# liuzuxin/FSRL

Hardware: AMD Instinct MI355X
Metric: policy-updates/sec (PPO-Lagrangian update(), SafetyCarCircle-v0 shape, 256x256 MLP, 20k-step buffer) (higher is better)
Workload: dtype f32; 1 GPU; configs[1] PPO-Lag update: repeat 4, clip 0.5, KL stop off, batch 256, N=20000 (20x1000), obs 8/act 2, 256x256; seeds_per_gpu=1, parallelism=independent agents x1

## Files before the change

fsrl_amd/_lib.py:

```python
import ctypes as C
import os

_HERE = os.path.dirname(os.path.abspath(__file__))
LIB_PATH = os.environ.get("FSRL_HIP_LIB") or os.path.join(_HERE, "libfsrl_hip.so")

FSRL_OK, FSRL_EINVAL, FSRL_ENOMEM, FSRL_EHIP, FSRL_ESTATE = 0, -22, -12, -5, -1
PPO_NSTATS = 11
ALGO_PPO_LAG, ALGO_TRPO_LAG, ALGO_CPO, ALGO_SAC_LAG, ALGO_FOCOPS = 0, 1, 2, 3, 4


class Config(C.Structure):
    _fields_ = [("algo", C.c_int32), ("obs_dim", C.c_int32), ("act_dim", C.c_int32),
                ("hidden", C.c_int32), ("n_critics", C.c_int32), ("env_num", C.c_int32),
                ("buffer_size", C.c_int64), ("max_action", C.c_float), ("gamma", C.c_double),
                ("gae_lambda", C.c_double), ("eps_clip", C.c_float), ("dual_clip", C.c_float),
                ("vf_coef", C.c_float), ("max_grad_norm", C.c_float), ("target_kl", C.c_float),
                ("norm_adv", C.c_int32), ("use_lagrangian", C.c_int32), ("lr", C.c_float),
                ("beta1", C.c_float), ("beta2", C.c_float), ("adam_eps", C.c_float), ("recompute_adv", C.c_int32),
                ("unbounded", C.c_int32), ("rew_norm", C.c_int32), ("value_clip", C.c_int32),
                ("hidden1", C.c_int32), ("hidden2", C.c_int32),
                ("n_hidden", C.c_int32), ("hidden_sizes", C.c_int32 * 8), ("force_layered", C.c_int32)]


class ShmEnv(C.Structure):
# ... 72 lines not shown
    "fsrl_store_push": (C.c_int, [_ctx, _i32, C.c_int32, _f, _f, _d, _d, _u8, _u8, _f, _i64, _d, _i32, _i64]),
    "fsrl_store_reset": (C.c_int, [_ctx, C.c_int]),
    "fsrl_store_len": (C.c_int64, [_ctx]),
    "fsrl_store_read": (C.c_int, [_ctx, _i64, C.c_int64, _f, _f, _d, _d, _u8, _u8, _f]),
    "fsrl_store_configure": (C.c_int, [_ctx, C.c_int64, C.c_int32]),
    "fsrl_store_geometry": (C.c_int, [_ctx, _i64, _i32]),
    "fsrl_store_sample0": (C.c_int, [_ctx, _i64, C.c_int64, _i64]),
    "fsrl_actor_forward": (C.c_int, [_ctx, _f, C.c_int32, _f, _f]),
    "fsrl_ppo_begin": (C.c_int, [_ctx, _d, C.c_double, C.c_int32, _i64]),
    "fsrl_ppo_pass": (C.c_int, [_ctx, _i64, C.c_uint64, _i32]),
    "fsrl_ppo_pass_result": (C.c_int, [_ctx, _i32]),
    "fsrl_ppo_end": (C.c_int, [_ctx, _f, C.c_int64, _i64]),
    "fsrl_ppo_update": (C.c_int, [_ctx, _d, C.c_double, C.c_int32, C.c_int32, _i64, C.c_uint64, _f,
                                  C.c_int64, _i64, _i32]),
    "fsrl_ppo_set_plan": (C.c_int, [_ctx, C.c_int32]),
    "fsrl_batch_get": (C.c_int, [_ctx, C.c_char_p, _f, C.c_int64]),
    "fsrl_group_create": (C.c_int, [_P(_ctx), C.c_int32, _P(_ctx)]),
    "fsrl_group_destroy": (C.c_int, [_ctx]),
    "fsrl_group_set_plan": (C.c_int, [_ctx, C.c_int32]),
    "fsrl_group_ppo_update": (C.c_int, [_ctx, _d, _d, C.c_int32, C.c_int32, _P(_i64), C.c_uint64, _P(_f), C.c_int64, _i64,
                                        _i32]),
    "fsrl_group_ppo_update_each": (C.c_int, [_ctx, _d, _d, _i32, _i32, _P(_i64), C.c_uint64, _P(_f), _i64, _i64, _i32]),
    "fsrl_group_collect_step": (C.c_int, [_ctx, _i32, _i32, _f, _f, _d, _d, _u8, _u8, _f, _i64, _d, _i32, _i64, _i32, _f, C.c_int32,
                                          C.c_int32, _f, _f, _f, _f]),
    "fsrl_group_actor_set_resident": (C.c_int, [_ctx, C.c_int32, C.c_double]),
    "fsrl_group_actor_resident_stats": (C.c_int, [_ctx, _i64]),
    "fsrl_group_actor_release": (C.c_int, [_ctx]),
    "fsrl_sac_group_create": (C.c_int, [_P(_ctx), C.c_int32, _P(_ctx)]),
    "fsrl_sac_group_destroy": (C.c_int, [_ctx]),
    "fsrl_sac_group_update": (C.c_int, [_ctx, C.c_int32, _i32, _d, _d]),
# ... 126 lines not shown
```

fsrl_amd/csrc/common.hpp:

```cpp
#pragma once
#include <hip/hip_runtime.h>
#include <stdint.h>

#include "../../include/fsrl_hip.h"

#define FSRL_MAX_NETS (1 + FSRL_MAX_CRITICS)
#define FSRL_TILE_M 16
#define FSRL_DOW 32
#define FSRL_MAX_OBS 128
#define FSRL_MAX_ACT 16
#define FSRL_W1_LDS 16
#define FSRL_RD 64
#define FSRL_RD_LOGP 16
#define FSRL_RD_ADV 17
#define FSRL_RD_RET 21
#define FSRL_RD_VOLD 25
#define FSRL_RD_MEAN 32
#define FSRL_RD_STD 48

typedef float f32x4 __attribute__((ext_vector_type(4)));
typedef float f32x2 __attribute__((ext_vector_type(2)));

struct NetOff {
    int sigma;
// ... 51 lines not shown
#define FSRL_PROBE(sa, n) false
#define FSRL_TS(buf, k) do { } while (0)
#endif

__device__ __forceinline__ void ppo_adam_math(const float g, float& m, float& v, float& p, const PpoStepArgs& sa) {
#pragma clang fp contract(off)
    m = fmaf(sa.one_minus_b1, g - m, m);
    v = v * sa.beta2;
    v = fmaf(sa.one_minus_b2 * g, g, v);
    const float denom = sqrtf(v) / sa.bc2_sqrt + sa.adam_eps;
    p = p + (-sa.step_size * m) / denom;
}

struct CtrlBlock {
    int stopped_after;
    int pad;
    double kl_sum;
    float last_grad_norm;
    float pad2;
};

__device__ __forceinline__ f32x4 mfma_16x16x4(float a, float b, f32x4 c) {
    return __builtin_amdgcn_mfma_f32_16x16x4f32(a, b, c, 0, 0, 0);
}

__device__ __forceinline__ f32x4 mfma_4x4x1(float a, float b, f32x4 c) {
    return __builtin_amdgcn_mfma_f32_4x4x1f32(a, b, c, 0, 0, 0);
}

__device__ __forceinline__ void store4_next(float* p, const f32x4 v) {
    asm volatile("global_store_dwordx4 %0, %1, off sc1\n\ts_nop 1" ::"v"(p), "v"(v) : "memory");
// ... 55 lines not shown
```

fsrl_amd/csrc/fsrl_hip.hip:

```cpp
#include <hip/hip_runtime.h>

#include <climits>
#include <cstddef>
#include <cmath>
#include <cstdarg>
#include <cstdio>
#include <cstdlib>
#include <cstring>
#include <algorithm>
#include <functional>
#include <string>
#include <vector>

#include "kernels_misc.hpp"
#include "kernels_mlp.hpp"
#include "kernels_fb.hpp"
#include "kernels_fbco.hpp"
#include "kernels_wgrad2.hpp"
#include "kernels_wgrad3.hpp"
#include "kernels_layered.hpp"
#include "kernels_focops_group.hpp"
#include "resident_ring.hpp"
#include "host_decisions.hpp"

// ... 74 lines not shown
    double* ret64 = nullptr; int64_t ret64_cap = 0;
    int64_t alloc_rows = 0;
    int active_envs = 0;
    std::vector<EnvBook> env;
    std::vector<uint8_t> h_flags;
    StorePtrs st{};
    static constexpr int STAGE_CAP = 4096;
    Staging stage[2];
    int cur_stage = 0;
    hipEvent_t store_ready = nullptr;

    BatchPtrs b{};
    int* d_indices = nullptr; uint8_t* d_end = nullptr; int* d_seg = nullptr;
    int* h_indices = nullptr; uint8_t* h_end = nullptr; int* h_seg = nullptr;
    float *values = nullptr, *vnext = nullptr, *advs = nullptr, *rets = nullptr, *logp_old = nullptr;
    int64_t N = 0;
    int n_seg = 0;
    bool batch_ready = false;

    int batch_size = 0, mbp_max = 0, n_tiles_max = 0;
    float *A1 = nullptr, *A2 = nullptr, *D1 = nullptr, *D2 = nullptr, *DO = nullptr;
    float *obs_p = nullptr, *rd_p = nullptr;
    float *statp = nullptr, *gsq_part = nullptr;
    int *d_perm = nullptr, *h_perm = nullptr;
    int *d_mbstart = nullptr, *d_mbsize = nullptr, *h_mbplan = nullptr;
    size_t mb_cap = 0;
    std::vector<int> mb_start, mb_size;
    float* d_stats = nullptr; int64_t stats_cap = 0;
    int64_t n_steps = 0;
    int pass_index = 0;
// ... 317 lines not shown
    lay_free(c);
    if (c->h_actor) (void)hipHostFree(c->h_actor);
    if (c->h_done) (void)hipHostFree(c->h_done);
    if (c->h_pa) (void)hipHostFree(c->h_pa);
    if (c->mbstat) (void)hipFree(c->mbstat);
    if (c->d_rms) (void)hipFree(c->d_rms);
    if (c->ret64) (void)hipFree(c->ret64);
    if (c->mu_old) (void)hipFree(c->mu_old);
    if (c->sigma_old) (void)hipFree(c->sigma_old);
    if (c->snap) (void)hipFree(c->snap);
    void* dptrs[] = {c->P, c->M, c->V, c->G, c->ctrl, c->st.obs, c->st.obs_next, c->st.act, c->st.rew,
                     c->st.cost, c->st.flags, c->b.obs, c->b.obs_next, c->b.act, c->b.rew, c->b.cost,
                     c->b.flags, c->d_indices, c->d_end, c->d_seg, c->values, c->vnext, c->advs,
                     c->rets, c->logp_old, c->A1, c->A2, c->D1, c->D2, c->DO, c->obs_p, c->rd_p, c->statp,
                     c->gsq_part, c->d_perm, c->d_mbstart, c->d_mbsize, c->d_stats,
                     c->scratch};
    for (void* p : dptrs) if (p) (void)hipFree(p);
    for (auto& pp : c->parts) if (pp.p) (void)hipFree(pp.p);
    void* hptrs[] = {c->h_ctrl, c->h_indices, c->h_end, c->h_seg, c->h_perm, c->h_mbplan};
    for (void* p : hptrs) if (p) (void)hipHostFree(p);
    for (auto& s : c->stage) {
        if (s.h) (void)hipHostFree(s.h);
        if (s.d) (void)hipFree(s.d);
        if (s.done) (void)hipEventDestroy(s.done);
    }
    for (hipEvent_t e : {c->store_ready, c->ev_a, c->ev_b, c->ev_c, c->perm_copied}) if (e) (void)hipEventDestroy(e);
    for (hipEvent_t e : c->k_ev) (void)hipEventDestroy(e);
    if (c->compute) (void)hipStreamDestroy(c->compute);
    if (c->side) (void)hipStreamDestroy(c->side);
    delete c;
    return 0;
}

extern "C" int fsrl_ctx_create(int device_id, const fsrl_config* cfg, fsrl_ctx** out) {
// ... 43 lines not shown
    CHECK_ARG(!cfg->rew_norm || cfg->algo != FSRL_ALGO_SAC_LAG, "reward_normalization acts on GAE returns: on-policy contexts only");
    int ndev = 0;
    HIPCHK(hipGetDeviceCount(&ndev));
    CHECK_ARG(device_id >= 0 && device_id < ndev, "device %d not present (%d devices)", device_id, ndev);
    HIPCHK(hipSetDevice(device_id));
    int n_cus_probe = 256;
    (void)hipDeviceGetAttribute(&n_cus_probe, hipDeviceAttributeMultiprocessorCount, device_id);
    fsrl_ctx* c = new fsrl_ctx();
    c->cfg = *cfg;
    c->cfg.hidden = Hpad_;
    c->h1 = h1_; c->h2 = h2_;
    c->device = device_id;
    c->n_cus = n_cus_probe > 0 ? n_cus_probe : 256;
    c->probe_tile16 = getenv("FSRL_TILE16") != nullptr;
    c->no_w2b_early = getenv("FSRL_NO_W2B_EARLY") != nullptr;
#ifdef FSRL_PROBES
    { const char* e = getenv("FSRL_DBG_PHASE"); c->probe_phase = e ? atoi(e) : 0; }
    { const char* e = getenv("FSRL_WGRAD_SKIP"); c->probe_wgrad_skip = e ? atoi(e) : 0; }
    c->no_spin = getenv("FSRL_NO_SPIN") != nullptr;
    c->no_xcd_pair = getenv("FSRL_NO_XCD_PAIR") != nullptr;
    c->no_fuse_adam = getenv("FSRL_NO_FUSE_ADAM") != nullptr;
    if (getenv("FSRL_TSTAMP")) {
        (void)hipMalloc(&c->probe_ts, 1024 * 16 * sizeof(unsigned long long));
        (void)hipMemset(c->probe_ts, 0, 1024 * 16 * sizeof(unsigned long long));
    }
#endif
    if (layered) lay_build_layout(c, cfg->hidden_sizes, cfg->n_hidden);
    else build_layout(c);
#define TRY(expr) do { hipError_t _e = (expr); if (_e != hipSuccess) { fail(FSRL_EHIP, "%s failed: %s", #expr, hipGetErrorString(_e)); fsrl_ctx_destroy(c); return FSRL_EHIP; } } while (0)
    TRY(hipStreamCreateWithFlags(&c->compute, hipStreamNonBlocking));
// ... 17 lines not shown
    c->h_flags.assign((size_t)c->alloc_rows, 0);
    const size_t ms = (size_t)c->alloc_rows;
    const int Do = cfg->obs_dim, Da = cfg->act_dim;
    TRY(hipMalloc(&c->st.obs, ms * Do * 4)); TRY(hipMalloc(&c->st.obs_next, ms * Do * 4));
    TRY(hipMalloc(&c->st.act, ms * Da * 4)); TRY(hipMalloc(&c->st.rew, ms * 8));
    TRY(hipMalloc(&c->st.cost, ms * 8)); TRY(hipMalloc(&c->st.flags, ms));
    TRY(hipMalloc(&c->b.obs, ms * Do * 4)); TRY(hipMalloc(&c->b.obs_next, ms * Do * 4));
    TRY(hipMalloc(&c->b.act, ms * Da * 4)); TRY(hipMalloc(&c->b.rew, ms * 8));
    TRY(hipMalloc(&c->b.cost, ms * 8)); TRY(hipMalloc(&c->b.flags, ms));
    TRY(hipMalloc(&c->d_indices, ms * 4)); TRY(hipMalloc(&c->d_end, ms)); TRY(hipMalloc(&c->d_seg, (ms + 2) * 4));
    TRY(hipHostMalloc(&c->h_indices, ms * 4)); TRY(hipHostMalloc(&c->h_end, ms)); TRY(hipHostMalloc(&c->h_seg, (ms + 2) * 4));
    const int C = cfg->n_critics;
    TRY(hipMalloc(&c->values, ms * C * 4)); TRY(hipMalloc(&c->vnext, ms * C * 4));
    TRY(hipMalloc(&c->advs, ms * C * 4)); TRY(hipMalloc(&c->rets, ms * C * 4));
    TRY(hipMalloc(&c->logp_old, ms * 4));
    TRY(hipMalloc(&c->d_perm, ms * 4)); TRY(hipHostMalloc(&c->h_perm, ms * 4));
    TRY(hipMalloc(&c->obs_p, (ms + 32) * Do * 4)); TRY(hipMemsetAsync(c->obs_p, 0, (ms + 32) * Do * 4, c->compute));
    TRY(hipMalloc(&c->rd_p, (ms + 32) * FSRL_RD * 4)); TRY(hipMemsetAsync(c->rd_p, 0, (ms + 32) * FSRL_RD * 4, c->compute));
    TRY(hipStreamSynchronize(c->compute));
    for (auto& s : c->stage) {
        const size_t k = fsrl_ctx::STAGE_CAP;
        TRY(hipHostMalloc(&s.h, k * stage_rec_bytes(Do, Da)));
        TRY(hipMalloc(&s.d, k * stage_rec_bytes(Do, Da)));
        TRY(hipEventCreateWithFlags(&s.done, hipEventDisableTiming));
    }
    TRY(hipEventCreateWithFlags(&c->store_ready, hipEventDisableTiming));
    TRY(hipEventCreate(&c->ev_a)); TRY(hipEventCreate(&c->ev_b)); TRY(hipEventCreate(&c->ev_c));
    TRY(hipEventCreateWithFlags(&c->perm_copied, hipEventDisableTiming));
    CtrlBlock init{INT_MAX, 0, 0.0, 0.0f, 0.0f};
    TRY(hipMemcpy(c->ctrl, &init, sizeof(init), hipMemcpyHostToDevice));
// ... 267 lines not shown
    rc = ensure_scratch(c, total);
    if (rc) return rc;
    std::vector<int> idx(N);
    for (size_t i = 0; i < N; ++i) {
        CHECK_ARG(indices[i] >= 0 && indices[i] < c->maxsize, "index %lld out of range", (long long)indices[i]);
        idx[i] = (int)indices[i];
    }
    char* base = (char*)c->scratch;
    hipStream_t s = c->compute;
    HIPCHK(hipMemcpyAsync(base + o_idx, idx.data(), N * 4, hipMemcpyHostToDevice, s));
    HIPCHK(hipMemsetAsync(base + o_end, 0, N, s));
    BatchPtrs b{(float*)(base + o_obs), (float*)(base + o_nxt), (float*)(base + o_act), (double*)(base + o_rew),
                (double*)(base + o_cost), (uint8_t*)(base + o_fl)};
    const size_t work = N * (2 * Do + Da + 1);
    hipLaunchKernelGGL(batch_gather_kernel, dim3((int)std::min<size_t>(2048, (work + 255) / 256)), dim3(256), 0, s, c->st, b,
                       (const int*)(base + o_idx), (const uint8_t*)(base + o_end), (int)n, (int)Do, (int)Da);
    HIPCHK(hipGetLastError());
    std::vector<uint8_t> fl(N);
    if (obs_out) HIPCHK(hipMemcpyAsync(obs_out, b.obs, N * Do * 4, hipMemcpyDeviceToHost, s));
    if (obs_next_out) HIPCHK(hipMemcpyAsync(obs_next_out, b.obs_next, N * Do * 4, hipMemcpyDeviceToHost, s));
    if (act_out) HIPCHK(hipMemcpyAsync(act_out, b.act, N * Da * 4, hipMemcpyDeviceToHost, s));
    if (rew_out) HIPCHK(hipMemcpyAsync(rew_out, b.rew, N * 8, hipMemcpyDeviceToHost, s));
    if (cost_out) HIPCHK(hipMemcpyAsync(cost_out, b.cost, N * 8, hipMemcpyDeviceToHost, s));
    HIPCHK(hipMemcpyAsync(fl.data(), b.flags, N, hipMemcpyDeviceToHost, s));
    HIPCHK(hipStreamSynchronize(s));
    for (size_t i = 0; i < N; ++i) {
        if (terminated_out) terminated_out[i] = fl[i] & 1;
        if (truncated_out) truncated_out[i] = (fl[i] >> 1) & 1;
    }
    return 0;
}
// ... 7 lines not shown
    }
    return fail(FSRL_EINVAL, "unsupported hidden width %d", H);
}

static int launch_infer(fsrl_ctx* c, const InferArgs& ia, int jobs_y, hipStream_t s) {
    const int tiles = (ia.N + 15) / 16;
    if (tiles == 0) return 0;
    if (c->lay) return lay_infer(c, ia, jobs_y, s);
    return dispatch_H(c->cfg.hidden, [&](auto hc) {
        constexpr int H = decltype(hc)::value;
        const int gx = std::min(tiles, std::max(1, c->n_cus / jobs_y));
        hipLaunchKernelGGL(mlp_infer_kernel<H>, dim3(gx, jobs_y), dim3(4 * H), 0, s, c->P, c->md, ia);
        HIPCHK(hipGetLastError());
        return 0;
    });
}

struct SacState;
static bool ctx_is_replay(const fsrl_ctx* c) { return c->cfg.algo == FSRL_ALGO_SAC_LAG; }
static int sac_actor_launch(fsrl_ctx* c, const float* h_obs, float* h_raw, int k);
static void sac_actor_finish(fsrl_ctx* c, const float* h_raw, int k, float* mu_out, float* sigma_out);
static int sac_raw_cols(const fsrl_ctx* c);
static bool sac_squashes(fsrl_ctx* c);
static bool sac_actor_resident_args(fsrl_ctx* c, const float** P, const ModelDesc** md);

struct PaLayout { unsigned long long* bell; unsigned* done; unsigned* state; float* obs; float* mu; float* sp; };
static PaLayout pa_layout(const fsrl_ctx* c) {
    char* b = (char*)c->h_pa;
    PaLayout l;
    l.bell = (unsigned long long*)b; l.done = (unsigned*)(b + 16); l.state = (unsigned*)(b + 32);
// ... 511 lines not shown
```

fsrl_amd/csrc/host_ppo.inc:

```
static int launch_gae(fsrl_ctx* c);
static int perm_upload(fsrl_ctx* c, int n, const int64_t* perm, uint64_t seed) {
    c->perm_tmp.resize((size_t)n);
    const PermFill pf = perm_fill(c->perm_tmp.data(), n, perm, c->shuffle_rng, seed);
    CHECK_ARG(pf.code != PERM_RANGE, "perm[%d]=%lld out of range", pf.index, pf.value);
    CHECK_ARG(pf.code != PERM_TWICE, "perm is not a permutation: %lld appears twice", pf.value);
    if (c->perm_in_flight) { HIPCHK(hipEventSynchronize(c->perm_copied)); c->perm_in_flight = false; }
    memcpy(c->h_perm, c->perm_tmp.data(), (size_t)n * 4);
    HIPCHK(hipMemcpyAsync(c->d_perm, c->h_perm, (size_t)n * 4, hipMemcpyHostToDevice, c->compute));
    HIPCHK(hipEventRecord(c->perm_copied, c->compute));
    c->perm_in_flight = true;
    return 0;
}

static int ensure_ppo_buffers(fsrl_ctx* c, int B) {
    const int mbp = round_up(2 * B, 32);
    if (mbp <= c->mbp_max) return 0;
    HIPCHK(hipStreamSynchronize(c->compute));
    for (float** p : {&c->A1, &c->A2, &c->D1, &c->D2, &c->DO, &c->statp, &c->gsq_part})
        if (*p) { HIPCHK(hipFree(*p)); *p = nullptr; }
    const int H = c->cfg.hidden, nn = c->md.n_nets;
    const size_t act = (size_t)nn * mbp * H * 4;
    HIPCHK(hipMalloc(&c->A1, act)); HIPCHK(hipMalloc(&c->A2, act));
    HIPCHK(hipMalloc(&c->D1, act)); HIPCHK(hipMalloc(&c->D2, act));
    HIPCHK(hipMalloc(&c->DO, (size_t)nn * mbp * FSRL_DOW * 4));
// ... 25 lines not shown
    for (int i = 0; i < FSRL_MAX_CRITICS; ++i) c->lagr[i] = 0.0;
    if (c->cfg.use_lagrangian && C > 1) {
        CHECK_ARG(lagrangians, "lags and values length must be equal");
        for (int i = 0; i < C - 1; ++i) c->lagr[i] = lagrangians[i];
    }
    c->rescaling = rescaling;
    c->batch_size = batch_size;
    const int64_t n = sample0(c, c->h_indices, c->h_end);
    c->N = n;
    if (n_out) *n_out = n;
    c->n_steps = 0;
    c->pass_index = 0;
    c->in_update = true;
    c->verdict_pending = false;
    c->t_fwdbwd_ms = 0; c->n_fwdbwd = 0; c->k_ev_used = 0;
    CtrlBlock init{INT_MAX, 0, 0.0, 0.0f, 0.0f};
    *c->h_ctrl = init;
    hipStream_t s = c->compute;
    HIPCHK(hipMemcpyAsync(c->ctrl, c->h_ctrl, sizeof(CtrlBlock), hipMemcpyHostToDevice, s));
    if (n == 0) { c->batch_ready = true; return 0; }
    int nseg = 0;
    c->h_seg[nseg++] = 0;
    for (int64_t i = 0; i + 1 < n; ++i) if (c->h_end[i]) c->h_seg[nseg++] = (int)i + 1;
    c->h_seg[nseg] = (int)n;
    HIPCHK(hipEventRecord(c->ev_a, s));
    HIPCHK(hipMemcpyAsync(c->d_indices, c->h_indices, (size_t)n * 4, hipMemcpyHostToDevice, s));
    HIPCHK(hipMemcpyAsync(c->d_end, c->h_end, (size_t)n, hipMemcpyHostToDevice, s));
    HIPCHK(hipMemcpyAsync(c->d_seg, c->h_seg, (size_t)(nseg + 1) * 4, hipMemcpyHostToDevice, s));
    const int Do = c->cfg.obs_dim, Da = c->cfg.act_dim;
    {
        const size_t work = (size_t)n * (2 * Do + Da + 1);
        const int blocks = (int)std::min<size_t>(2048, (work + 255) / 256);
        hipLaunchKernelGGL(batch_gather_kernel, dim3(blocks), dim3(256), 0, s, c->st, c->b, c->d_indices,
                           c->d_end, (int)n, Do, Da);
        HIPCHK(hipGetLastError());
    }
    InferArgs ia{};
    ia.obs = c->b.obs; ia.obs_next = c->b.obs_next; ia.act = c->b.act; ia.flags = c->b.flags;
    ia.values = c->values; ia.vnext = c->vnext; ia.logp_old = c->logp_old; ia.mu_out = nullptr;
    if (c->cfg.algo == FSRL_ALGO_FOCOPS) {
        if (!c->mu_old) {
            HIPCHK(hipMalloc(&c->mu_old, (size_t)c->alloc_rows * Da * 4));
            HIPCHK(hipMalloc(&c->sigma_old, FSRL_MAX_ACT * 4));
        }
        ia.mu_out = c->mu_old;
        HIPCHK(hipMemcpyAsync(c->sigma_old, c->P + c->md.net[0].sigma, (size_t)Da * 4, hipMemcpyDeviceToDevice, s));
    }
    ia.N = (int)n; ia.C = C; ia.max_action = c->cfg.max_action;
    rc = launch_infer(c, ia, 2 * C + 1, s);
    if (rc) return rc;
    c->n_seg = nseg;
    rc = launch_gae(c);
    if (rc) return rc;
    HIPCHK(hipEventRecord(c->ev_b, s));
    split_plan((int)n, batch_size, c->mb_start, c->mb_size);
    const int bs_rows = (int)std::min<int64_t>(batch_size, std::max<int64_t>(n, 1));
    rc = c->lay ? lay_ensure_mb(c, bs_rows) : ensure_ppo_buffers(c, bs_rows);
    if (rc) return rc;
    const size_t nmb = c->mb_start.size();
    if (nmb > c->mb_cap) {
        HIPCHK(hipStreamSynchronize(s));
        if (c->d_mbstart) HIPCHK(hipFree(c->d_mbstart));
        if (c->d_mbsize) HIPCHK(hipFree(c->d_mbsize));
        if (c->h_mbplan) HIPCHK(hipHostFree(c->h_mbplan));
// ... 31 lines not shown
    HIPCHK(hipGetLastError());
    if (c->cfg.rew_norm) {
        hipLaunchKernelGGL(ret_rms_update_kernel, dim3(c->cfg.n_critics), dim3(1024), 0, c->compute, c->ret64, c->d_rms,
                           (int)c->N);
        HIPCHK(hipGetLastError());
    }
    return 0;
}

static int ppo_recompute_advantages(fsrl_ctx* c) {
    const int C = c->cfg.n_critics;
    InferArgs ia{};
    ia.obs = c->b.obs; ia.obs_next = c->b.obs_next; ia.act = nullptr; ia.flags = c->b.flags;
    ia.values = c->values; ia.vnext = c->vnext; ia.logp_old = nullptr; ia.mu_out = nullptr;
    ia.N = (int)c->N; ia.C = C; ia.max_action = c->cfg.max_action;
    int rc = launch_infer(c, ia, 2 * C, c->compute);
    if (rc) return rc;
    return launch_gae(c);
}

static int ensure_stats(fsrl_ctx* c, int64_t steps) {
    if (steps <= c->stats_cap) return 0;
    int64_t cap = std::max<int64_t>(steps, c->stats_cap * 2);
    cap = std::max<int64_t>(cap, 1024);
    float* nw = nullptr;
    HIPCHK(hipMalloc(&nw, (size_t)cap * FSRL_PPO_NSTATS * 4));
    if (c->d_stats) {
        HIPCHK(hipStreamSynchronize(c->compute));
        HIPCHK(hipMemcpy(nw, c->d_stats, (size_t)c->stats_cap * FSRL_PPO_NSTATS * 4, hipMemcpyDeviceToDevice));
        HIPCHK(hipFree(c->d_stats));
    }
// ... 265 lines not shown
    CHECK_ARG(c, "null ctx");
    CHECK_ARG(repeat >= 0, "repeat must be >= 0");
    int64_t n = 0;
    int rc = fsrl_ppo_begin(c, lagrangians, rescaling, batch_size, &n);
    if (rc) return rc;
    if (stopped_pass_out) *stopped_pass_out = -1;
    for (int k = 0; k < repeat; ++k) {
        int32_t stopped = 0;
        rc = fsrl_ppo_pass(c, perms ? perms + (size_t)k * n : nullptr, seed ? seed + k : 0, &stopped);
        if (rc) { c->in_update = false; return rc; }
        if (stopped) { if (stopped_pass_out) *stopped_pass_out = k; break; }
    }
    return fsrl_ppo_end(c, stats_out, cap_steps, n_steps_out);
}

extern "C" int fsrl_batch_get(fsrl_ctx* c, const char* which, float* out, int64_t cap) {
    CHECK_ARG(c && which && out, "null argument");
    if (!c->batch_ready) return fail(FSRL_ESTATE, "no batch: call fsrl_ppo_begin first");
    ENTER_DEV(c);
    const int64_t n = c->N;
    const int C = c->cfg.n_critics;
    const float* src = nullptr;
    int cols = C;
    if (!strcmp(which, "values")) src = c->values;
    else if (!strcmp(which, "rets")) src = c->rets;
    else if (!strcmp(which, "advs")) src = c->advs;
    else if (!strcmp(which, "vnext")) src = c->vnext;
    else if (!strcmp(which, "logp_old")) { src = c->logp_old; cols = 1; }
    else return fail(FSRL_EINVAL, "unknown batch field '%s'", which);
    CHECK_ARG(cap >= n * cols, "out too small");
// ... 8 lines not shown
```

fsrl_amd/csrc/kernels_misc.hpp:

```cpp
#pragma once
#include "common.hpp"

struct StorePtrs {
    float* obs;
    float* obs_next;
    float* act;
    double* rew;
    double* cost;
    uint8_t* flags;
};

__global__ void store_scatter_kernel(StorePtrs st, const uint8_t* __restrict__ recs, const int rec, int k, int Do, int Da) {
    const int per = 2 * Do + Da + 1;
    for (int e = blockIdx.x * blockDim.x + threadIdx.x; e < k * per; e += gridDim.x * blockDim.x) {
        const int row = e / per, f = e - row * per;
        const uint8_t* r = recs + (size_t)row * rec;
        const size_t dst = (size_t)*reinterpret_cast<const int*>(r + 16);
        const float* x = reinterpret_cast<const float*>(r + 24);
        if (f < Do) st.obs[dst * Do + f] = x[f];
        else if (f < 2 * Do) st.obs_next[dst * Do + (f - Do)] = x[f];
        else if (f < 2 * Do + Da) st.act[dst * Da + (f - 2 * Do)] = x[f];
        else {
            st.rew[dst] = *reinterpret_cast<const double*>(r);
            st.cost[dst] = *reinterpret_cast<const double*>(r + 8);
            st.flags[dst] = (uint8_t)*reinterpret_cast<const uint32_t*>(r + 20);
        }
    }
}

struct BatchPtrs {
    float* obs; float* obs_next; float* act; double* rew; double* cost; uint8_t* flags;
};

__global__ void batch_gather_kernel(StorePtrs st, BatchPtrs b, const int* __restrict__ indices,
                                    const uint8_t* __restrict__ end_flag, int n, int Do, int Da) {
    const int per = 2 * Do + Da + 1;
    for (size_t e = (size_t)blockIdx.x * blockDim.x + threadIdx.x; e < (size_t)n * per;
         e += (size_t)gridDim.x * blockDim.x) {
        const int row = (int)(e / per), f = (int)(e - (size_t)row * per);
        const size_t src = (size_t)indices[row];
        if (f < Do) b.obs[(size_t)row * Do + f] = st.obs[src * Do + f];
        else if (f < 2 * Do) b.obs_next[(size_t)row * Do + (f - Do)] = st.obs_next[src * Do + (f - Do)];
        else if (f < 2 * Do + Da) b.act[(size_t)row * Da + (f - 2 * Do)] = st.act[src * Da + (f - 2 * Do)];
        else {
            b.rew[row] = st.rew[src];
            b.cost[row] = st.cost[src];
            b.flags[row] = (uint8_t)((st.flags[src] & 3) | (end_flag[row] ? 4 : 0));
        }
    }
}

struct GaeArgs {
    const float* values;
    const float* vnext;
    const double* rew;
    const double* cost;
    const uint8_t* flags;
    const int* seg_start;
    float* advs;
    float* rets;
    double* adv64;
    int N;
    double gamma, gl;
    const double* rms;
// ... 284 lines not shown
```

fsrl_amd/csrc/kernels_mlp.hpp:

```cpp
#pragma once
#include <type_traits>
#include "common.hpp"

__host__ __device__ constexpr int tile_rows(int R) { return R > 16 ? R : 16; }

template <int H, int ROWS = 16>
struct TileSmem {
    static constexpr int LD = H + 4;
    static constexpr int XK = (ROWS > 16) ? 64 : FSRL_MAX_OBS;
    float xT[XK * ROWS];
    float h1[ROWS * LD];
    float h2[ROWS * LD];
    float d2[ROWS * LD];
    float out[ROWS * FSRL_MAX_ACT];
    float dout[ROWS * FSRL_DOW];
    float rd[ROWS * FSRL_RD];
    float st[ROWS * 4];
    float w3[FSRL_MAX_ACT * H];
    float b1[H], b2[H], b3[FSRL_MAX_ACT], sig[FSRL_MAX_ACT];
    float w1[H * FSRL_W1_LDS];
};

template <int H>
struct TileGeom {
// ... 401 lines not shown
        __syncthreads();
#pragma unroll
        for (int u = 0; u < NX; ++u) {
            const int e = tid + u * NT;
            if (e < 16 * Do) { const int i = div_by_magic((unsigned)e, magic), k = e - i * Do; sm.xT[k * 16 + i] = xn[u]; }
        }
        tile = ntile; row0 = nrow0; n_valid = nn_valid;
    }
    if (a.done) {
        if (tid < min(NT, max(256, (16 * a.raw_cols + 63) & ~63))) __atomic_thread_fence(__ATOMIC_RELEASE);
        __syncthreads();
        if (tid == 0) __hip_atomic_store(a.done + blockIdx.x, a.seq, __ATOMIC_RELAXED, __HIP_MEMORY_SCOPE_SYSTEM);
    }
}

#define PACTOR_BLOCKS 4
struct PActorArgs {
    const float* obs;
    float* mu_out;
    float* sigma_param_out;
    const unsigned long long* bell;
    unsigned* done;
    unsigned* state;
    unsigned gen, last_seq;
    unsigned long long timeout_ticks;
    float max_action;
    int raw_cols;
};
#define PACTOR_EXIT 0xFFFFFFFFu

// ... 988 lines not shown
```

fsrl_amd/engine.py:

```python
import ctypes as C
from dataclasses import dataclass
from typing import Optional, Sequence

import numpy as np

from . import _lib

_f32p, _f64p = C.POINTER(C.c_float), C.POINTER(C.c_double)
_u8p, _i32p, _i64p = C.POINTER(C.c_uint8), C.POINTER(C.c_int32), C.POINTER(C.c_int64)


def _ptr(a, t):
    return a.ctypes.data_as(t) if a is not None else None


@dataclass
class EngineConfig:
    obs_dim: int = 8
    act_dim: int = 2
    hidden: int = 128
    hidden_sizes: Optional[Sequence[int]] = None
    force_layered: bool = False
    n_critics: int = 2
    env_num: int = 20
# ... 341 lines not shown
        return bool(stopped.value)

    def ppo_end(self):
        n = C.c_int64()
        _lib.check(self.lib.fsrl_ppo_end(self._ctx, None, 0, C.byref(n)))
        return n.value

    def ppo_end_stats(self, max_steps: int):
        n = C.c_int64()
        out = np.empty((max(max_steps, 1), _lib.PPO_NSTATS), np.float32)
        _lib.check(self.lib.fsrl_ppo_end(self._ctx, _ptr(out, _f32p), out.shape[0], C.byref(n)))
        return out[:n.value]

    def ppo_set_plan(self, tall_tiles: int = -1):
        _lib.check(self.lib.fsrl_ppo_set_plan(self._ctx, int(tall_tiles)))

    def ppo_update(self, lagrangians, rescaling, batch_size, repeat, perms=None, seed=0):
        n = self.ppo_begin(lagrangians, rescaling, batch_size)
        stopped_pass = -1
        steps_per_pass = max(1, -(-n // max(batch_size, 1)))
        try:
            for k in range(repeat):
                if self.ppo_pass(None if perms is None else perms[k], seed + k if seed else 0):
                    stopped_pass = k
                    break
            stats = self.ppo_end_stats(steps_per_pass * max(repeat, 1))
        except BaseException:
            self.ppo_abort()
            raise
        return stats, stopped_pass
# ... 593 lines not shown
```

include/fsrl_hip.h:

```cpp
#ifndef FSRL_HIP_H
#define FSRL_HIP_H

#include <stdint.h>

#ifdef __cplusplus
extern "C" {
#endif

#define FSRL_OK 0
#define FSRL_EINVAL (-22)
#define FSRL_ENOMEM (-12)
#define FSRL_EHIP (-5)
#define FSRL_ESTATE (-1)

#define FSRL_ALGO_PPO_LAG 0
#define FSRL_ALGO_TRPO_LAG 1
#define FSRL_ALGO_CPO 2
#define FSRL_ALGO_SAC_LAG 3
#define FSRL_ALGO_FOCOPS 4

#define FSRL_MAX_CRITICS 4
#define FSRL_MAX_HIDDEN 8
#define FSRL_MAX_WIDTH 4096
#define FSRL_PPO_NSTATS 11
// ... 110 lines not shown
int fsrl_actor_release(fsrl_ctx* ctx);

int fsrl_store_sizes(const fsrl_ctx* ctx, int64_t* sizes_out, int32_t n);

int fsrl_ppo_begin(fsrl_ctx* ctx, const double* lagrangians, double rescaling,
                   int32_t batch_size, int64_t* n_out);
int fsrl_ppo_pass(fsrl_ctx* ctx, const int64_t* perm, uint64_t seed, int32_t* stopped_out);
int fsrl_ppo_pass_result(fsrl_ctx* ctx, int32_t* stopped_out);
int fsrl_ppo_end(fsrl_ctx* ctx, float* stats_out, int64_t cap_steps, int64_t* n_steps_out);
int fsrl_ppo_abort(fsrl_ctx* ctx);
int fsrl_ppo_update(fsrl_ctx* ctx, const double* lagrangians, double rescaling,
                    int32_t batch_size, int32_t repeat, const int64_t* perms, uint64_t seed,
                    float* stats_out, int64_t cap_steps, int64_t* n_steps_out,
                    int32_t* stopped_pass_out);

int fsrl_ppo_set_plan(fsrl_ctx* ctx, int32_t tall_tiles);

typedef struct fsrl_group fsrl_group;
int fsrl_group_create(fsrl_ctx** ctxs, int32_t k, fsrl_group** out);
int fsrl_group_destroy(fsrl_group* group);
int fsrl_group_set_plan(fsrl_group* group, int32_t tall_tiles);
int fsrl_group_ppo_update(fsrl_group* group, const double* lagrangians, const double* rescaling, int32_t batch_size,
                          int32_t repeat, const int64_t* const* perms, uint64_t seed, float* const* stats_out,
                          int64_t cap_steps, int64_t* n_steps_out, int32_t* stopped_pass_out);
int fsrl_group_ppo_update_each(fsrl_group* group, const double* lagrangians, const double* rescaling, const int32_t* batch_sizes,
                               const int32_t* repeats, const int64_t* const* perms, uint64_t seed, float* const* stats_out,
                               const int64_t* cap_steps, int64_t* n_steps_out, int32_t* stopped_pass_out);
int fsrl_group_collect_step(fsrl_group* group, const int32_t* k, const int32_t* env_ids, const float* obs, const float* act,
                            const double* rew, const double* cost, const uint8_t* terminated, const uint8_t* truncated,
                            const float* obs_next, int64_t* ptr_out, double* ep_rew_out, int32_t* ep_len_out,
// ... 186 lines not shown
```

Before: 130.9 updates/s.

## Reuse next-row critic values for V(s') instead of a second dense critic pass

During PPO batch preparation, the gather kernel now checks, bitwise, whether each row's obs_next equals the next row's obs. Rows where they match (not episode end, not last) take vnext straight from values[i+1] in a small fill kernel. Only the mismatched rows are listed and sent through a sparse critic forward, which cuts the dense inference jobs from 2C+1 to C+1. In exchange, the gather kernel gains ballots, atomics and a stamp array, and an extra kernel launch is added. It also assumes that a forward pass on equal inputs gives bitwise-equal outputs.

```diff
diff --git a/fsrl_amd/_lib.py b/fsrl_amd/_lib.py
--- a/fsrl_amd/_lib.py
+++ b/fsrl_amd/_lib.py
@@ -110,6 +110,7 @@
     "fsrl_ppo_update": (C.c_int, [_ctx, _d, C.c_double, C.c_int32, C.c_int32, _i64, C.c_uint64, _f,
                                   C.c_int64, _i64, _i32]),
     "fsrl_ppo_set_plan": (C.c_int, [_ctx, C.c_int32]),
+    "fsrl_ppo_vnext_uncovered": (C.c_int, [_ctx, _i64]),
     "fsrl_batch_get": (C.c_int, [_ctx, C.c_char_p, _f, C.c_int64]),
     "fsrl_group_create": (C.c_int, [_P(_ctx), C.c_int32, _P(_ctx)]),
     "fsrl_group_destroy": (C.c_int, [_ctx]),
diff --git a/fsrl_amd/csrc/common.hpp b/fsrl_amd/csrc/common.hpp
--- a/fsrl_amd/csrc/common.hpp
+++ b/fsrl_amd/csrc/common.hpp
@@ -89,7 +89,7 @@
 
 struct CtrlBlock {
     int stopped_after;
-    int pad;
+    int vnext_unc;
     double kl_sum;
     float last_grad_norm;
     float pad2;
diff --git a/fsrl_amd/csrc/fsrl_hip.hip b/fsrl_amd/csrc/fsrl_hip.hip
--- a/fsrl_amd/csrc/fsrl_hip.hip
+++ b/fsrl_amd/csrc/fsrl_hip.hip
@@ -112,6 +112,9 @@
     int* d_indices = nullptr; uint8_t* d_end = nullptr; int* d_seg = nullptr;
     int* h_indices = nullptr; uint8_t* h_end = nullptr; int* h_seg = nullptr;
     float *values = nullptr, *vnext = nullptr, *advs = nullptr, *rets = nullptr, *logp_old = nullptr;
+    unsigned* vn_stamp = nullptr; int* vn_list = nullptr; unsigned vn_epoch = 0; int* h_vn_count = nullptr;
+    bool vn_reuse = false;
+    bool no_vnext_reuse = false;
     int64_t N = 0;
     int n_seg = 0;
     bool batch_ready = false;
@@ -459,10 +462,10 @@
                      c->b.flags, c->d_indices, c->d_end, c->d_seg, c->values, c->vnext, c->advs,
                      c->rets, c->logp_old, c->A1, c->A2, c->D1, c->D2, c->DO, c->obs_p, c->rd_p, c->statp,
                      c->gsq_part, c->d_perm, c->d_mbstart, c->d_mbsize, c->d_stats,
-                     c->scratch};
+                     c->scratch, c->vn_stamp, c->vn_list};
     for (void* p : dptrs) if (p) (void)hipFree(p);
     for (auto& pp : c->parts) if (pp.p) (void)hipFree(pp.p);
-    void* hptrs[] = {c->h_ctrl, c->h_indices, c->h_end, c->h_seg, c->h_perm, c->h_mbplan};
+    void* hptrs[] = {c->h_ctrl, c->h_indices, c->h_end, c->h_seg, c->h_perm, c->h_mbplan, c->h_vn_count};
     for (void* p : hptrs) if (p) (void)hipHostFree(p);
     for (auto& s : c->stage) {
         if (s.h) (void)hipHostFree(s.h);
@@ -536,6 +539,7 @@
     c->n_cus = n_cus_probe > 0 ? n_cus_probe : 256;
     c->probe_tile16 = getenv("FSRL_TILE16") != nullptr;
     c->no_w2b_early = getenv("FSRL_NO_W2B_EARLY") != nullptr;
+    c->no_vnext_reuse = getenv("FSRL_NO_VNEXT_REUSE") != nullptr;
 #ifdef FSRL_PROBES
     { const char* e = getenv("FSRL_DBG_PHASE"); c->probe_phase = e ? atoi(e) : 0; }
     { const char* e = getenv("FSRL_WGRAD_SKIP"); c->probe_wgrad_skip = e ? atoi(e) : 0; }
@@ -583,6 +587,8 @@
     TRY(hipMalloc(&c->values, ms * C * 4)); TRY(hipMalloc(&c->vnext, ms * C * 4));
     TRY(hipMalloc(&c->advs, ms * C * 4)); TRY(hipMalloc(&c->rets, ms * C * 4));
     TRY(hipMalloc(&c->logp_old, ms * 4));
+    TRY(hipMalloc(&c->vn_stamp, ms * 4)); TRY(hipMemsetAsync(c->vn_stamp, 0, ms * 4, c->compute)); TRY(hipMalloc(&c->vn_list, ms * 4));
+    TRY(hipHostMalloc(&c->h_vn_count, sizeof(int))); *c->h_vn_count = -1;
     TRY(hipMalloc(&c->d_perm, ms * 4)); TRY(hipHostMalloc(&c->h_perm, ms * 4));
     TRY(hipMalloc(&c->obs_p, (ms + 32) * Do * 4)); TRY(hipMemsetAsync(c->obs_p, 0, (ms + 32) * Do * 4, c->compute));
     TRY(hipMalloc(&c->rd_p, (ms + 32) * FSRL_RD * 4)); TRY(hipMemsetAsync(c->rd_p, 0, (ms + 32) * FSRL_RD * 4, c->compute));
@@ -880,7 +886,7 @@
                 (double*)(base + o_cost), (uint8_t*)(base + o_fl)};
     const size_t work = N * (2 * Do + Da + 1);
     hipLaunchKernelGGL(batch_gather_kernel, dim3((int)std::min<size_t>(2048, (work + 255) / 256)), dim3(256), 0, s, c->st, b,
-                       (const int*)(base + o_idx), (const uint8_t*)(base + o_end), (int)n, (int)Do, (int)Da);
+                       (const int*)(base + o_idx), (const uint8_t*)(base + o_end), (int)n, (int)Do, (int)Da, VnextCover{});
     HIPCHK(hipGetLastError());
     std::vector<uint8_t> fl(N);
     if (obs_out) HIPCHK(hipMemcpyAsync(obs_out, b.obs, N * Do * 4, hipMemcpyDeviceToHost, s));
@@ -918,6 +924,26 @@
         HIPCHK(hipGetLastError());
         return 0;
     });
+}
+
+static int launch_infer_reuse(fsrl_ctx* c, const InferArgs& ia, int n_dense, hipStream_t s) {
+    const int tiles = (ia.N + 15) / 16;
+    if (tiles == 0) return 0;
+    const VnextCover vc{c->vn_stamp, c->vn_list, &c->ctrl->vnext_unc, c->vn_epoch};
+    int rc = dispatch_H(c->cfg.hidden, [&](auto hc) {
+        constexpr int H = decltype(hc)::value;
+        const int64_t want = (int64_t)tiles * n_dense;
+        const int G = (int)std::max<int64_t>(n_dense, std::min<int64_t>(c->n_cus, want));
+        hipLaunchKernelGGL(ppo_infer_kernel<H>, dim3(G), dim3(4 * H), 0, s, c->P, c->md, ia, n_dense, vc.list, vc.count);
+        HIPCHK(hipGetLastError());
+        return 0;
+    });
+    if (rc) return rc;
+    const int work = ia.N * ia.C;
+    hipLaunchKernelGGL(vnext_fill_kernel, dim3((work + 255) / 256), dim3(256), 0, s, vc, ia.values, ia.vnext, ia.flags, ia.N, ia.C,
+                       c->h_vn_count);
+    HIPCHK(hipGetLastError());
+    return 0;
 }
 
 struct SacState;
diff --git a/fsrl_amd/csrc/host_ppo.inc b/fsrl_amd/csrc/host_ppo.inc
--- a/fsrl_amd/csrc/host_ppo.inc
+++ b/fsrl_amd/csrc/host_ppo.inc
@@ -63,6 +63,8 @@
     c->in_update = true;
     c->verdict_pending = false;
     c->t_fwdbwd_ms = 0; c->n_fwdbwd = 0; c->k_ev_used = 0;
+    c->vn_reuse = !c->lay && !c->group && !c->no_vnext_reuse;
+    *c->h_vn_count = (c->vn_reuse && n == 0) ? 0 : -1;
     CtrlBlock init{INT_MAX, 0, 0.0, 0.0f, 0.0f};
     *c->h_ctrl = init;
     hipStream_t s = c->compute;
@@ -77,11 +79,19 @@
     HIPCHK(hipMemcpyAsync(c->d_end, c->h_end, (size_t)n, hipMemcpyHostToDevice, s));
     HIPCHK(hipMemcpyAsync(c->d_seg, c->h_seg, (size_t)(nseg + 1) * 4, hipMemcpyHostToDevice, s));
     const int Do = c->cfg.obs_dim, Da = c->cfg.act_dim;
+    VnextCover vc{};
+    if (c->vn_reuse) {
+        if (++c->vn_epoch == 0) {
+            HIPCHK(hipMemsetAsync(c->vn_stamp, 0, (size_t)c->alloc_rows * 4, s));
+            c->vn_epoch = 1;
+        }
+        vc = VnextCover{c->vn_stamp, c->vn_list, &c->ctrl->vnext_unc, c->vn_epoch};
+    }
     {
         const size_t work = (size_t)n * (2 * Do + Da + 1);
         const int blocks = (int)std::min<size_t>(2048, (work + 255) / 256);
         hipLaunchKernelGGL(batch_gather_kernel, dim3(blocks), dim3(256), 0, s, c->st, c->b, c->d_indices,
-                           c->d_end, (int)n, Do, Da);
+                           c->d_end, (int)n, Do, Da, vc);
         HIPCHK(hipGetLastError());
     }
     InferArgs ia{};
@@ -96,7 +106,7 @@
         HIPCHK(hipMemcpyAsync(c->sigma_old, c->P + c->md.net[0].sigma, (size_t)Da * 4, hipMemcpyDeviceToDevice, s));
     }
     ia.N = (int)n; ia.C = C; ia.max_action = c->cfg.max_action;
-    rc = launch_infer(c, ia, 2 * C + 1, s);
+    rc = c->vn_reuse ? launch_infer_reuse(c, ia, C + 1, s) : launch_infer(c, ia, 2 * C + 1, s);
     if (rc) return rc;
     c->n_seg = nseg;
     rc = launch_gae(c);
@@ -158,7 +168,7 @@
     ia.obs = c->b.obs; ia.obs_next = c->b.obs_next; ia.act = nullptr; ia.flags = c->b.flags;
     ia.values = c->values; ia.vnext = c->vnext; ia.logp_old = nullptr; ia.mu_out = nullptr;
     ia.N = (int)c->N; ia.C = C; ia.max_action = c->cfg.max_action;
-    int rc = launch_infer(c, ia, 2 * C, c->compute);
+    int rc = c->vn_reuse ? launch_infer_reuse(c, ia, C, c->compute) : launch_infer(c, ia, 2 * C, c->compute);
     if (rc) return rc;
     return launch_gae(c);
 }
@@ -454,6 +464,14 @@
     return fsrl_ppo_end(c, stats_out, cap_steps, n_steps_out);
 }
 
+extern "C" int fsrl_ppo_vnext_uncovered(fsrl_ctx* c, int64_t* out) {
+    CHECK_ARG(c && out, "null argument");
+    ENTER_DEV(c);
+    if (c->in_update) HIPCHK(hipStreamSynchronize(c->compute));
+    *out = *c->h_vn_count;
+    return 0;
+}
+
 extern "C" int fsrl_batch_get(fsrl_ctx* c, const char* which, float* out, int64_t cap) {
     CHECK_ARG(c && which && out, "null argument");
     if (!c->batch_ready) return fail(FSRL_ESTATE, "no batch: call fsrl_ppo_begin first");
diff --git a/fsrl_amd/csrc/kernels_misc.hpp b/fsrl_amd/csrc/kernels_misc.hpp
--- a/fsrl_amd/csrc/kernels_misc.hpp
+++ b/fsrl_amd/csrc/kernels_misc.hpp
@@ -32,22 +32,71 @@
     float* obs; float* obs_next; float* act; double* rew; double* cost; uint8_t* flags;
 };
 
+struct VnextCover {
+    unsigned* stamp;
+    int* list;
+    int* count;
+    unsigned epoch;
+};
+__device__ __forceinline__ bool vnext_uncover(const VnextCover& vc, int row) {
+    return atomicExch(vc.stamp + row, vc.epoch) != vc.epoch;
+}
+
 __global__ void batch_gather_kernel(StorePtrs st, BatchPtrs b, const int* __restrict__ indices,
-                                    const uint8_t* __restrict__ end_flag, int n, int Do, int Da) {
+                                    const uint8_t* __restrict__ end_flag, int n, int Do, int Da, const VnextCover vc) {
+    __shared__ int s_found, s_base;
     const int per = 2 * Do + Da + 1;
-    for (size_t e = (size_t)blockIdx.x * blockDim.x + threadIdx.x; e < (size_t)n * per;
-         e += (size_t)gridDim.x * blockDim.x) {
-        const int row = (int)(e / per), f = (int)(e - (size_t)row * per);
-        const size_t src = (size_t)indices[row];
-        if (f < Do) b.obs[(size_t)row * Do + f] = st.obs[src * Do + f];
-        else if (f < 2 * Do) b.obs_next[(size_t)row * Do + (f - Do)] = st.obs_next[src * Do + (f - Do)];
-        else if (f < 2 * Do + Da) b.act[(size_t)row * Da + (f - 2 * Do)] = st.act[src * Da + (f - 2 * Do)];
-        else {
-            b.rew[row] = st.rew[src];
-            b.cost[row] = st.cost[src];
-            b.flags[row] = (uint8_t)((st.flags[src] & 3) | (end_flag[row] ? 4 : 0));
-        }
-    }
+    const size_t total = (size_t)n * per;
+    for (size_t e0 = (size_t)blockIdx.x * blockDim.x; e0 < total; e0 += (size_t)gridDim.x * blockDim.x) {
+        const size_t e = e0 + threadIdx.x;
+        int found = -1;
+        if (vc.stamp) {
+            if (threadIdx.x == 0) s_found = 0;
+            __syncthreads();
+        }
+        if (e < total) {
+            const int row = (int)(e / per), f = (int)(e - (size_t)row * per);
+            const size_t src = (size_t)indices[row];
+            if (f < Do) b.obs[(size_t)row * Do + f] = st.obs[src * Do + f];
+            else if (f < 2 * Do) {
+                const int k = f - Do;
+                const float v = st.obs_next[src * Do + k];
+                b.obs_next[(size_t)row * Do + k] = v;
+                if (vc.stamp) {
+                    const bool differs = row + 1 < n && !end_flag[row] &&
+                                         __float_as_uint(v) != __float_as_uint(st.obs[(size_t)indices[row + 1] * Do + k]);
+                    const unsigned long long m = __ballot(differs);
+                    const int lane = threadIdx.x & 63, lo = max(lane - k, 0), hi = min(lane + (Do - 1 - k), 63);
+                    const unsigned long long seg = (hi - lo == 63) ? ~0ull : (((1ull << (hi - lo + 1)) - 1ull) << lo);
+                    if (lane == lo && (m & seg) != 0 && vnext_uncover(vc, row)) found = row;
+                }
+            }
+            else if (f < 2 * Do + Da) b.act[(size_t)row * Da + (f - 2 * Do)] = st.act[src * Da + (f - 2 * Do)];
+            else {
+                b.rew[row] = st.rew[src];
+                b.cost[row] = st.cost[src];
+                b.flags[row] = (uint8_t)((st.flags[src] & 3) | (end_flag[row] ? 4 : 0));
+                if (vc.stamp && (row + 1 >= n || end_flag[row]) && vnext_uncover(vc, row)) found = row;
+            }
+        }
+        if (vc.stamp) {
+            const int slot = found >= 0 ? atomicAdd(&s_found, 1) : 0;
+            __syncthreads();
+            if (threadIdx.x == 0 && s_found > 0) s_base = atomicAdd(vc.count, s_found);
+            __syncthreads();
+            if (found >= 0) vc.list[s_base + slot] = found;
+        }
+    }
+}
+
+__global__ void vnext_fill_kernel(const VnextCover vc, const float* __restrict__ values, float* __restrict__ vnext,
+                                  const uint8_t* __restrict__ flags, int n, int C, int* __restrict__ h_count) {
+    const int e = blockIdx.x * blockDim.x + threadIdx.x;
+    if (e == 0 && h_count) __hip_atomic_store(h_count, *vc.count, __ATOMIC_RELAXED, __HIP_MEMORY_SCOPE_SYSTEM);
+    if (e >= n * C) return;
+    const int c = e / n, i = e - c * n;
+    if (vc.stamp[i] == vc.epoch || i + 1 >= n) return;
+    vnext[(size_t)c * n + i] = (flags[i] & 1) ? 0.0f : values[(size_t)c * n + i + 1];
 }
 
 struct GaeArgs {
diff --git a/fsrl_amd/csrc/kernels_mlp.hpp b/fsrl_amd/csrc/kernels_mlp.hpp
--- a/fsrl_amd/csrc/kernels_mlp.hpp
+++ b/fsrl_amd/csrc/kernels_mlp.hpp
@@ -439,6 +439,100 @@
     }
 }
 
+template <int H>
+__device__ __forceinline__ void ppo_infer_job(TileSmem<H>& sm, const float* __restrict__ P, const ModelDesc& md, const InferArgs& a,
+                                              const int net, const bool is_actor, const int c, const int bx, const int gx,
+                                              const int* __restrict__ list, const int n_rows) {
+    constexpr int NT = TileGeom<H>::NT;
+    constexpr int NX = TileStage<H>::NX;
+    const int tid = threadIdx.x;
+    const NetOff no = md.net[net];
+    const int Do = md.Do;
+    const int n_tiles = (n_rows + 15) >> 4;
+    if (bx >= n_tiles) return;
+    const unsigned magic = div_magic(Do);
+    const float* __restrict__ X = list ? a.obs_next : a.obs;
+    auto load_x = [&](const int row0, const int n_valid, const int e) -> float {
+        if (e >= n_valid * Do) return 0.0f;
+        if (!list) return X[(size_t)row0 * Do + e];
+        const int i = div_by_magic((unsigned)e, magic), k = e - i * Do;
+        return X[(size_t)list[row0 + i] * Do + k];
+    };
+    int tile = bx, row0 = tile * 16, n_valid = min(16, n_rows - row0);
+    TileStage<H> stg;
+    stg.issue_params(P, no, Do, md.Da, tid);
+#pragma unroll
+    for (int u = 0; u < NX; ++u) stg.xv[u] = load_x(row0, n_valid, tid + u * NT);
+#pragma unroll
+    for (int u = 0; u < TileStage<H>::NR; ++u) stg.rdv[u] = 0.0f;
+    FwdW2Frag<H> wf;
+    wf.load(P + no.W2f, tid >> 6, tid & 63);
+    stg.commit(sm, no, Do, tid);
+    while (true) {
+        const int ntile = tile + gx;
+        const int nrow0 = ntile * 16, nn_valid = min(16, n_rows - nrow0);
+        float xn[NX];
+        if (ntile < n_tiles) {
+#pragma unroll
+            for (int u = 0; u < NX; ++u) xn[u] = load_x(nrow0, nn_valid, tid + u * NT);
+        }
+        __syncthreads();
+        tile_forward<H>(sm, P, no, Do, tid, wf);
+        if (tid < n_valid) {
+            if (!is_actor) {
+                float v = sm.out[tid * FSRL_MAX_ACT];
+                if (list) {
+                    const int r = list[row0 + tid];
+                    if (a.flags[r] & 1) v = 0.0f;
+                    a.vnext[(size_t)c * a.N + r] = v;
+                } else {
+                    a.values[(size_t)c * a.N + row0 + tid] = v;
+                }
+            } else {
+                const int r = row0 + tid;
+                float logp = 0.0f;
+                for (int d = 0; d < md.Da; ++d) {
+                    const float x = sm.out[tid * FSRL_MAX_ACT + d];
+                    const float mu = md.unbounded ? x : a.max_action * tanhf(x);
+                    const float sig = expf(sm.sig[d]);
+                    if (a.mu_out) a.mu_out[(size_t)r * md.Da + d] = mu;
+                    if (a.act) {
+                        const float diff = a.act[(size_t)r * md.Da + d] - mu;
+                        logp += -(diff * diff) / (2.0f * sig * sig) - logf(sig) - LOG_SQRT_2PI;
+                    }
+                }
+                if (a.logp_old) a.logp_old[r] = logp;
+            }
+        }
+        if (ntile >= n_tiles) break;
+        __syncthreads();
+#pragma unroll
+        for (int u = 0; u < NX; ++u) {
+            const int e = tid + u * NT;
+            if (e < 16 * Do) { const int i = div_by_magic((unsigned)e, magic), k = e - i * Do; sm.xT[k * 16 + i] = xn[u]; }
+        }
+        tile = ntile; row0 = nrow0; n_valid = nn_valid;
+    }
+    __syncthreads();
+}
+
+template <int H>
+__global__ __launch_bounds__(4 * H) void ppo_infer_kernel(const float* __restrict__ P, const ModelDesc md, const InferArgs a,
+                                                         const int n_dense, const int* __restrict__ unc_list,
+                                                         const int* __restrict__ unc_count) {
+    __shared__ TileSmem<H> sm;
+    const int b = blockIdx.x, G = gridDim.x, C = a.C;
+    {
+        const int job = b % n_dense;
+        ppo_infer_job<H>(sm, P, md, a, job == C ? 0 : 1 + job, job == C, job, b / n_dense, (G - job + n_dense - 1) / n_dense, nullptr, a.N);
+    }
+    {
+        const int c = b % C;
+        const int n_unc = min(max(*unc_count, 0), a.N);
+        ppo_infer_job<H>(sm, P, md, a, 1 + c, false, c, b / C, (G - c + C - 1) / C, unc_list, n_unc);
+    }
+}
+
 #define PACTOR_BLOCKS 4
 struct PActorArgs {
     const float* obs;
diff --git a/fsrl_amd/engine.py b/fsrl_amd/engine.py
--- a/fsrl_amd/engine.py
+++ b/fsrl_amd/engine.py
@@ -379,6 +379,11 @@
 
     def ppo_set_plan(self, tall_tiles: int = -1):
         _lib.check(self.lib.fsrl_ppo_set_plan(self._ctx, int(tall_tiles)))
+
+    def ppo_vnext_uncovered(self) -> int:
+        n = C.c_int64()
+        _lib.check(self.lib.fsrl_ppo_vnext_uncovered(self._ctx, C.byref(n)))
+        return n.value
 
     def ppo_update(self, lagrangians, rescaling, batch_size, repeat, perms=None, seed=0):
         n = self.ppo_begin(lagrangians, rescaling, batch_size)
diff --git a/include/fsrl_hip.h b/include/fsrl_hip.h
--- a/include/fsrl_hip.h
+++ b/include/fsrl_hip.h
@@ -148,6 +148,8 @@
                     float* stats_out, int64_t cap_steps, int64_t* n_steps_out,
                     int32_t* stopped_pass_out);
 
+int fsrl_ppo_vnext_uncovered(fsrl_ctx* ctx, int64_t* out);
+
 int fsrl_ppo_set_plan(fsrl_ctx* ctx, int32_t tall_tiles);
 
 typedef struct fsrl_group fsrl_group;
```

New measurement: 135.0 updates/s (median of 5 runs). +3.1%, better.
